# Stylish-TTS/stylish-tts

Hardware: AMD Instinct MI355X
Metric: audio frames/sec/GPU (24 kHz) forward+backward; DDP scaling 1/2/4/8 MI355X (higher is better)
Workload: dtype bf16 GEMM operands, f32 accumulation/storage; 1 GPU; c3: B=32/GPU T=520 frames (6.5 s) L=100

## Files before the change

stylish_tts_amd/csrc/bwd.hip:

```cpp
#include "sty_common.h"

namespace sty {

__device__ __forceinline__ double wave_sum(double v) {
  for (int o = 32; o > 0; o >>= 1) v += __shfl_xor(v, o);
  return v;
}

template <int N>
__device__ __forceinline__ void block_sum(double (&v)[N], double (*red)[4]) {
  const int lane = threadIdx.x & 63, wave = threadIdx.x >> 6;
#pragma unroll
  for (int i = 0; i < N; ++i) {
    v[i] = wave_sum(v[i]);
    if (lane == 0) red[i][wave] = v[i];
  }
  __syncthreads();
  if (threadIdx.x == 0) {
#pragma unroll
    for (int i = 0; i < N; ++i) v[i] = red[i][0] + red[i][1] + red[i][2] + red[i][3];
  }
}

__global__ __launch_bounds__(256) void pro_bwd_kernel(int mode_, const float* __restrict__ u, int Cu, int cu0,
// ... 542 lines not shown
  const float om = (in && out_mask) ? out_mask[(size_t)b * T + t] : 1.f;
  float mean = 0.f;
#pragma unroll
  for (int c = 0; c < 32; ++c) mean += xv[c];
  mean *= (1.0f / 32.0f);
  float var = 0.f;
#pragma unroll
  for (int c = 0; c < 32; ++c) {
    xv[c] -= mean;
    var = fmaf(xv[c], xv[c], var);
  }
  const float r = 1.0f / sqrtf(var * (1.0f / 32.0f) + eps);
  float s1 = 0.f, s2 = 0.f;
#pragma unroll
  for (int c = 0; c < 32; ++c) {
    xv[c] *= r;
    gv[c] *= om;
    const float dxh = gv[c] * A_s[c];
    s1 += dxh;
    s2 = fmaf(dxh, xv[c], s2);
  }
  s1 *= (1.0f / 32.0f);
  s2 *= (1.0f / 32.0f);
  if (in) {
#pragma unroll
    for (int c = 0; c < 32; ++c) {
      const float d = r * (gv[c] * A_s[c] - s1 - xv[c] * s2);
      if (h16 & 4) {
        sty_st_any(dx, base + (size_t)c * T, d, true);
      } else {
        float* o = reinterpret_cast<float*>(dx) + base + (size_t)c * T;
        *o = accumulate ? *o + d : d;
      }
    }
  }
#pragma unroll
  for (int c = 0; c < 32; ++c) {
    const float a0 = sty_half_sum_to_lane31(gv[c] * xv[c]);
    const float a1 = sty_half_sum_to_lane31(gv[c]);
    if ((tid & 31) == 31) {
      atomicAdd(&red[c], a0);
      atomicAdd(&red[32 + c], a1);
    }
  }
  __syncthreads();
  if (tid < 64) part[((size_t)b * gridDim.x + blockIdx.x) * 64 + tid] = red[tid];
}
__global__ __launch_bounds__(64) void chan_ln32_param_sum_kernel(const float* __restrict__ part, int B, int nblk, int ada,
                                                                 float* __restrict__ dgb, float* __restrict__ dw,
                                                                 float* __restrict__ db) {
  const int i = blockIdx.x, lane = threadIdx.x;
  const int slot = ada ? (i & 63) : i, b0 = ada ? i >> 6 : 0, nb = ada ? 1 : B;
  double s = 0.0;
  for (int b = b0; b < b0 + nb; ++b)
    for (int k = lane; k < nblk; k += 64) s += (double)part[((size_t)b * nblk + k) * 64 + slot];
  s = wave_sum(s);
  if (lane == 0) {
    if (ada)
      dgb[(size_t)b0 * 64 + slot] += (float)s;
    else if (slot < 32)
      dw[slot] += (float)s;
    else
      db[slot - 32] += (float)s;
  }
}

__global__ void cast_any_kernel(const void* __restrict__ x, size_t n, void* __restrict__ y, int to16) {
  const size_t i = (size_t)blockIdx.x * 256 + threadIdx.x;
  if (i < n) sty_st_any(y, i, sty_ld_any(x, i, !to16), to16);
}
int launch_cast_f32_to_16(const float* x, size_t n, void* y16, hipStream_t st) {
  hipLaunchKernelGGL(cast_any_kernel, dim3((unsigned)((n + 255) / 256)), dim3(256), 0, st, x, n, y16, 1);
  STY_LAUNCH_CHECK();
  return STY_OK;
}
int launch_cast_16_to_f32(const void* x16, size_t n, float* y, hipStream_t st) {
  hipLaunchKernelGGL(cast_any_kernel, dim3((unsigned)((n + 255) / 256)), dim3(256), 0, st, x16, n, y, 0);
  STY_LAUNCH_CHECK();
  return STY_OK;
}
bool chan_ln32_eligible(int B, int C, int T, int relu) {
  return C == 32 && !relu && (size_t)B * T >= 65536 && getenv("STY_NO_LN32_BWD") == nullptr;
}
int launch_chan_ln_bwd(const float* x, const float* dy, const float* y, int B, int C, int T, float eps, int ada,
                       const float* w, const float* gb, int relu, const float* out_mask, float* dx, int accumulate,
                       float* mu_tmp, float* r_tmp, float* dgb, float* dw, float* db, hipStream_t st, int h16) {
  const bool no32 = getenv("STY_NO_LN32_BWD") != nullptr;
  if (C == 32 && !relu && (size_t)B * T >= 65536 && !no32) {
    const int nblk = cdiv(T, 256);
    if ((h16 & 4) && accumulate) {
      set_error("chan_ln_bwd: a two-byte dx cannot be accumulated into");
      return STY_EINVAL;
    }
    hipLaunchKernelGGL(chan_ln32_bwd_kernel, dim3(nblk, B), dim3(256), 0, st, x, dy, T, eps, ada, w, gb, out_mask, dx, accumulate,
                       mu_tmp, h16);
    hipLaunchKernelGGL(chan_ln32_param_sum_kernel, dim3(ada ? B * 64 : 64), dim3(64), 0, st, mu_tmp, B, nblk, ada, dgb, dw, db);
    STY_LAUNCH_CHECK();
    return STY_OK;
  }
  if (h16) {
    set_error("chan_ln_bwd: two-byte tensors only on the C = 32 long-row kernel (chan_ln32_eligible)");
    return STY_EINVAL;
  }
  if ((size_t)B * T < 65536 && C <= 256)
    hipLaunchKernelGGL((chan_ln_bwd_dx_reg_kernel<16, 16>), dim3(cdiv(T, 16), B), dim3(256), 0, st, x, dy, y, C, T, eps, ada, w,
                       gb, relu, out_mask, dx, accumulate, mu_tmp, r_tmp);
  else if ((size_t)B * T >= 65536)
    hipLaunchKernelGGL(chan_ln_bwd_dx_kernel<64>, dim3(cdiv(T, 64), B), dim3(256), 0, st, x, dy, y, C, T, eps, ada, w, gb,
                       relu, out_mask, dx, accumulate, mu_tmp, r_tmp);
  else
    hipLaunchKernelGGL(chan_ln_bwd_dx_kernel<16>, dim3(cdiv(T, 16), B), dim3(256), 0, st, x, dy, y, C, T, eps, ada, w, gb,
                       relu, out_mask, dx, accumulate, mu_tmp, r_tmp);
  hipLaunchKernelGGL(chan_ln_bwd_param_kernel, dim3(C, B), dim3(256), 0, st, x, dy, y, mu_tmp, r_tmp, C, T, ada, relu,
                     out_mask, dgb, dw, db);
  STY_LAUNCH_CHECK();
  return STY_OK;
}

__global__ __launch_bounds__(256) void grn_bwd_kernel(const double* __restrict__ part, int nseg,
                                                      const float* __restrict__ gamma,
                                                      const float* __restrict__ ds, int C4,
                                                      float* __restrict__ coef, float* __restrict__ dgamma) {
  __shared__ float gxs[1024];
  __shared__ double red[2][4];
  const int b = blockIdx.x;
  if (nseg < 32) {
    for (int c = threadIdx.x; c < C4; c += 256) {
      double sq = 0.0;
      for (int k = 0; k < nseg; ++k) sq += part[(((size_t)b * C4 + c) * nseg + k) * 2 + 1];
      gxs[c] = (float)sqrt(sq);
    }
  } else {
    const int lane = threadIdx.x & 63, wave = threadIdx.x >> 6;
    for (int c = wave; c < C4; c += 4) {
      const double* pp = part + ((size_t)b * C4 + c) * nseg * 2 + 1;
      double sq = 0.0;
      for (int k = lane; k < nseg; k += 64) sq += pp[(size_t)k * 2];
      for (int o = 32; o > 0; o >>= 1) sq += __shfl_xor(sq, o);
      if (lane == 0) gxs[c] = (float)sqrt(sq);
    }
  }
  __syncthreads();
  double acc[1] = {0.0};
  for (int c = threadIdx.x; c < C4; c += 256) acc[0] += gxs[c];
  __shared__ float mean_s, dot_s;
  block_sum<1>(acc, red);
  if (threadIdx.x == 0) mean_s = (float)(acc[0] / C4);
  __syncthreads();
  const float m = mean_s + 1e-6f;
  double d2[1] = {0.0};
  for (int c = threadIdx.x; c < C4; c += 256) {
    const float dnx = ds[(size_t)b * C4 + c] * gamma[c];
    d2[0] += (double)dnx * gxs[c];
    atomicAdd(&dgamma[c], ds[(size_t)b * C4 + c] * (gxs[c] / m));
  }
  __syncthreads();
  block_sum<1>(d2, red);
  if (threadIdx.x == 0) dot_s = (float)d2[0];
  __syncthreads();
  for (int c = threadIdx.x; c < C4; c += 256) {
    const float dnx = ds[(size_t)b * C4 + c] * gamma[c];
    const float dgx = dnx / m - dot_s / (m * m) / (float)C4;
    coef[(size_t)b * C4 + c] = gxs[c] > 0.f ? dgx / gxs[c] : 0.f;
  }
}
int launch_grn_bwd(const double* part, int nseg, const float* gamma, const float* ds, int B, int C4, float* coef,
                   float* dgamma, hipStream_t st) {
  if (C4 > 1024) {
    set_error("grn_bwd: 4C > 1024");
    return STY_EINVAL;
  }
  hipLaunchKernelGGL(grn_bwd_kernel, dim3(B), dim3(256), 0, st, part, nseg, gamma, ds, C4, coef, dgamma);
  STY_LAUNCH_CHECK();
  return STY_OK;
}

__global__ void act_fwd_kernel(int kind, const float* __restrict__ x, const float* __restrict__ alpha, int C, int T,
                               float* __restrict__ y) {
  const int t = blockIdx.x * 256 + threadIdx.x, c = blockIdx.y, b = blockIdx.z;
  if (t >= T) return;
  if (kind == ACT_GLU) {
    const float a = x[((size_t)b * 2 * C + c) * T + t], g = x[((size_t)b * 2 * C + C + c) * T + t];
    y[((size_t)b * C + c) * T + t] = a / (1.f + expf(-g));
    return;
  }
  const size_t o = ((size_t)b * C + c) * T + t;
  const float v = x[o];
  float r = v;
  if (kind == ACT_RELU) r = fmaxf(v, 0.f);
  else if (kind == ACT_SWISH) r = v / (1.f + expf(-v));
  else if (kind == ACT_SNAKE) r = sty_snake(v, alpha[c], 1.f / alpha[c]);
  else if (kind == 100) r = tanhf(v);
  else if (kind == ACT_GELU) r = 0.5f * v * (1.0f + erff(v * 0.70710678118654752f));
  y[o] = r;
}
__device__ __forceinline__ float act_apply1(int kind, float v, float al, float ral) {
  float r = v;
// ... 787 lines not shown
```

stylish_tts_amd/csrc/model.h:

```cpp
#pragma once
#include <string>
#include <unordered_map>
#include <vector>

#include "sty_common.h"

namespace sty {

struct Param {
  const float* p = nullptr;
  std::vector<int64_t> shape;
};

int convnext32_ntiles(int T);
int launch_convnext32(const Cnx32Args& a, int B, int pass, hipStream_t st);
int launch_pack_w2a(const float* w2, const float* b2, const float* grn_beta, int C, float* w2a, float* b2eff,
                    hipStream_t st);
int launch_attention(const AttnArgs& a, int B, int DH, hipStream_t st);
int launch_rope_n(float* q, float* k, int B, int H, int DH, int L, int d, hipStream_t st, float sgn = 1.0f);
int launch_style_expand(const float* style, int B, int S, int L, float* y, hipStream_t st);
int launch_row_sum_add(const float* src, int rows, int L, float* dst, hipStream_t st);
int launch_wn_dw_bwd(const float* dw, const float* g, const float* v, int C, int K, float* dg, float* dv, hipStream_t st);
int launch_dur_post_bwd(const float* d, const float* mask, const float* go, int B, int NC, int L, float* gd, hipStream_t st);
int trainer_duration_forward(struct Trainer* t, int B, int L, const int64_t* texts, const int64_t* lengths, const float* style,
// ... 159 lines not shown
  int heads = 2;
};

struct Trainer;
struct StyleResBlk {
  int Cin = 0, Cout = 0;
  bool down = false, has_sc = false;
  PackedConv c1, c2, sc;
  const float* dw_w9 = nullptr;
  const float* dw_b = nullptr;
};
struct StylePlan {
  int n_mels = 80, style_dim = 64;
  PackedConv stem;
  StyleResBlk blk[4];
  PackedConv head;
  const float *fc_w = nullptr, *fc_b = nullptr;
};

}

struct sty_model {
  std::string kind;
  std::unordered_map<std::string, sty::Param> params;
  std::vector<std::string> requested;
  bool finalized = false, prepared = false;
  bool train_prepared = false;
  hipEvent_t prepared_ev = nullptr;
  int style_dim = 64;
  char* arena = nullptr;
  size_t arena_bytes = 0;
  sty::Bump ab;
  std::vector<sty::PackJob> jobs;
  std::vector<sty::StyleFcDesc> fcs;
  sty::StyleFcDesc* fcs_dev = nullptr;
  size_t gb_floats_per_batch = 0;
  std::string missing;
  sty::VocoderPlan voc;
  sty::TextEncPlan te;
  sty::DecoderPlan dec;
  sty::StylePlan sty_enc;
  sty::DurationPlan dur;
  sty::PitchEnergyPlan pe;
  sty::PackedConv pse_pre;
  float* stft_default = nullptr;
  bool train_enabled = false;
  char* garena = nullptr;
  std::unordered_map<const float*, float*> pgrad;
  std::unordered_map<std::string, float*> pgrad_by_key;
  std::unordered_map<const float*, sty::PackedConv> dgrad;
  std::unordered_map<const float*, sty::PackedConv> plain_of;
  void* fcs_bwd_dev = nullptr;
  sty::MultiJob* mj_dev[5] = {nullptr, nullptr, nullptr, nullptr, nullptr};
  int* mj_blk_dev[5] = {nullptr, nullptr, nullptr, nullptr, nullptr};
  int mj_nblk[5] = {0, 0, 0, 0, 0};
  int* mj_blk1_dev = nullptr;
  int mj_nblk1 = 0, mj_nsn = 0;
  bool mj_ready = false;
  size_t seg_job_split = 0;
  int seg_blk_split = 0;
  sty_grad_hook grad_hook = nullptr;
  void* grad_hook_user = nullptr;
  sty_train_opts topts = {0, 0, 0, 0, 0.1f, 0u, 0.2f, 0, 0};
  struct sty::Trainer* trainer = nullptr;
};

#include <functional>
#include <unordered_set>
namespace sty {
int launch_pro_bwd(int mode, const float* u, int Cu, int cu0, const float* x, int B, int C, int T, const float* pa,
                   const float* ps, int pC, int pc0, const float* alpha, const float* mask, float* dx, int accumulate,
                   float* dpa, float* dps, float* dalpha, hipStream_t st);
int launch_adain_fold_bwd(const float* da, const float* ds, const float* mean, const float* rstd, const float* gb, int B,
                          int C, int T, float* dgb, float* c0, float* c1, hipStream_t st);
int launch_row_axpb(const float* x, const float* c0, const float* c1, int rows, int T, float* dx, hipStream_t st);
int launch_pro_bwd_adain(const void* u, int uh, const void* x, int xh, int B, int C, int T, const float* pa, const float* ps,
                         const float* alpha, const float* mean, const float* rstd, const float* gb, void* dx, int dh,
                         int accumulate, float* dgb, float* dalpha, int hw, hipStream_t st, const void* dsrc = nullptr);
int launch_adain_stats(const double* part, int nseg, int rows, int T, float eps, float* mean, float* rstd,
                       hipStream_t st);
int launch_cast_f32_to_16(const float* x, size_t n, void* y16, hipStream_t st);
int launch_cast_16_to_f32(const void* x16, size_t n, float* y, hipStream_t st);
bool chan_ln32_eligible(int B, int C, int T, int relu);
int launch_chan_ln_bwd(const float* x, const float* dy, const float* y, int B, int C, int T, float eps, int ada,
                       const float* w, const float* gb, int relu, const float* out_mask, float* dx, int accumulate,
                       float* mu_tmp, float* r_tmp, float* dgb, float* dw, float* db, hipStream_t st, int h16 = 0);
int launch_grn_bwd(const double* part, int nseg, const float* gamma, const float* ds, int B, int C4, float* coef,
                   float* dgamma, hipStream_t st);
int launch_act_fwd(int kind, const float* x, const float* alpha, int B, int C, int T, float* y, hipStream_t st);
int launch_act_bwd(int kind, const float* x, const float* dy, const float* alpha, int B, int C, int T, float* dx,
                   int accumulate, float* dalpha, hipStream_t st);
int launch_row_scale_add(const float* src, const float* coef, float k, int rows, int T, float* dst, hipStream_t st);
int launch_dwconv_fwd(const float* x, const float* w, const float* bias, int B, int C, int T, int K, int pad, float* y,
                      hipStream_t st);
size_t dwconv_bwd_scratch_floats(int B, int C, int T, int K);
int launch_dwconv_bwd(const float* x, const float* dy, const float* w, int B, int C, int T, int K, int pad, float* dx,
                      int accumulate, float* dw, float* db, float* scratch, hipStream_t st, const float* dx_src = nullptr,
                      int x16 = 0, int dy16 = 0);
int launch_bn_eval_fwd(const float* x, const float* w, const float* b, const float* rm, const float* rv, float eps,
                       int B, int C, int T, float* y, hipStream_t st);
int launch_bn_eval_bwd(const float* x, const float* dy, const float* w, const float* rm, const float* rv, float eps,
                       int B, int C, int T, float* dx, float* dw, float* db, hipStream_t st);
size_t bias_grad_scratch_floats(int B, int C, int T);
int launch_bias_grad(const float* g, const float* mask, int B, int C, int T, int shuffle, float scale, float* db,
                     float* scratch, hipStream_t st);
int launch_style_fc_bwd(const void* descs_dev, int nlayers, int B, int style_dim, const float* style,
                        const float* dgb_base, float* dstyle, hipStream_t st);
int launch_istft64_bwd(int B, int F, const float* audio, const float* daudio, const float* logamp, const float* real,
                       const float* imag, const float* bbr, const float* bbi, float* dlogamp, float* dreal,
                       float* dimag, hipStream_t st);
size_t wgrad_partial_floats(const PackedConv& w, int B, int T);
struct WgReduceDefer;
WgReduceDefer* wgrad_defer_create();
void wgrad_defer_destroy(WgReduceDefer* d);
WgReduceDefer* wgrad_defer_set(WgReduceDefer* d);
size_t wgrad_defer_pending(const WgReduceDefer* d);
int wgrad_defer_flush(WgReduceDefer* d, int site, hipStream_t st);
inline bool wgrad_fuses_bias(const PackedConv& w) { return w.K <= 12; }
int launch_conv1d_wgrad(const ConvArgs& fwd, const float* g, const float* gmask, float scale, float* gwp,
                        float* partial, float* gbias, bool* bias_done, hipStream_t st);
bool conv1d_wgrad_reads_twins_only(const ConvArgs& fwd, bool gmask);
int launch_pack_dgrad(const float* wp, int K, int CinP, int CoutP, float* wd, hipStream_t st);
int launch_b2eff_bwd(const float* g, const float* w2, const float* beta, int C, float* db2, float* dbeta, float* dW2,
                     hipStream_t st);
int launch_unpack_grad(const float* gwp, const float* g, const float* v, int Cout, int Cin, int K, int CinP, int CoutP,
                       int glu, float* dW, float* dg, float* dv, hipStream_t st);
int launch_attention_bwd(const AttnArgs& a, const float* dO, float* dQ, float* dK, float* dV, size_t dqbs, size_t dkbs,
                         size_t dvbs, size_t dobs, int B, int DH, float* ws, hipStream_t st, int overwrite = 0);
bool attention_bwd_can_overwrite(const AttnArgs& a, int DH);
bool attention_bwd_mfma_dh(int DH);
size_t attention_bwd_ws_floats(int B, int H, int T);
int launch_rope_signed(float* q, float* k, int B, int H, int DH, int L, int d, const float* theta4, float sgn,
                       hipStream_t st);
int launch_embedding_bwd(const int64_t* tokens, const float* g, int B, int L, int H, int ntok, float scale, float* demb,
                         hipStream_t st);
int launch_bmm_ct_bwd(const float* g, const float* ali, int B, int C, int L, int T, float* denc, hipStream_t st);
int launch_slice_add(const float* src, int Csrc, int c0, int B, int C, int T, float* dst, hipStream_t st);
int launch_fnv_bwd(const float* pitch, const float* energy, const float* voiced, const float* w34, const float* g, int B,
                   int T, float* dw34, float* dp, float* de, float* dv, hipStream_t st);
int launch_fnv_unpack(const float* dw34, const float* g0, const float* v0, const float* g1, const float* v1,
                      const float* g2, const float* v2, float* dg0, float* dv0, float* db0, float* dg1, float* dv1,
                      float* db1, float* dg2, float* dv2, float* db2, hipStream_t st);
int launch_pack_dgrad2d(const float* wp, int KW, int KH, int Cin, int Cout, int CinP, int CoutP, int CinPd, int CoutPd,
                        float* wd, hipStream_t st);
size_t dwconv2d_s2_bwd_scratch_floats(int B, int C, int H, int W);
int launch_dwconv2d_s2_bwd(const float* x, const float* gy, const float* gate, const float* w9, int B, int C, int H, int W, float* dx,
                           int accumulate, float* dw9, float* db, float* scratch, hipStream_t st, __bf16* dx16 = nullptr,
                           const float* mask16 = nullptr);
int launch_pad_cols(const float* x, size_t rows, int W, float* y, hipStream_t st);
int launch_flat_mask(int B, int H, int Wp, int Hv, int Wv, float* m, hipStream_t st);
int launch_dw2d_sn_unpack(const float* g9, const float* w, const float* u, const float* v, const float* t, int C,
                          float* dW, hipStream_t st);
int launch_avgpool2_bwd(const float* gy, int BC, int H, int W, float scale, float* dx, const float* gate, hipStream_t st,
                        __bf16* dx16 = nullptr, const float* mask16 = nullptr, int C = 0);
int launch_pool_fc_bwd(const float* x, int B, int C, int n, int count, const float* W, int S, const float* gs,
                       float* dW, float* db, float* dx, int accumulate, hipStream_t st);
int launch_bn_train_fwd(const float* x, const float* w, const float* b, float* rm, float* rv, float eps, float momentum,
                        int B, int C, int T, float* y, float* mean, float* rstd, double* part, hipStream_t st);
int launch_bn_train_bwd(const float* x, const float* dy, const float* w, const float* mean, const float* rstd, int B,
                        int C, int T, float* dx, int accumulate, float* dw, float* db, float* sums, hipStream_t st);
int launch_dropout(const float* x, const float* res, size_t n, float p, unsigned seed, unsigned site, float* y,
                   int accumulate, hipStream_t st, size_t group = 1);
int launch_box_smooth(const float* x, int B, int T, int width, float* y, int accumulate, hipStream_t st);
size_t sn_power_iter_scratch_floats(int Cout, int n);
int trainer_style_forward(struct Trainer* t, int B, int T, const float* mel, float* style, void* ws, size_t ws_bytes,
                          hipStream_t st, size_t* need, const float* pitch = nullptr, const float* energy = nullptr);
int trainer_style_backward(struct Trainer* t, const float* d_style, hipStream_t st);
int trainer_style_tap(struct Trainer* t, int i, int grad, float* dst, int* C, int* H, int* W, hipStream_t st);
struct Trainer;
// ... 21 lines not shown
```

stylish_tts_amd/csrc/sty_common.h:

```cpp
#pragma once
#include <hip/hip_runtime.h>
#include <stdint.h>
#include <stdio.h>

#include "../../include/stylish_hip.h"

namespace sty {

void set_error(const char* fmt, ...);
int hip_fail(hipError_t e, const char* what);

#define STY_HIP(expr)                                      \
  do {                                                     \
    hipError_t _e = (expr);                                \
    if (_e != hipSuccess) return sty::hip_fail(_e, #expr); \
  } while (0)

#define STY_LAUNCH_CHECK() STY_HIP(hipGetLastError())

extern thread_local const void* g_last_kernel;
template <class R, class... A>
inline const void* kernel_handle(R (*f)(A...)) {
  return reinterpret_cast<const void*>(f);
}
// ... 30 lines not shown
  r[6] = (__bf16)v6;
  r[7] = (__bf16)v7;
  return r;
}
#endif

#ifdef __HIPCC__
typedef __bf16 bf16x2 __attribute__((ext_vector_type(2)));
__device__ __forceinline__ float sty_bf_lo(unsigned u) { return __builtin_bit_cast(float, u << 16); }
__device__ __forceinline__ float sty_bf_hi(unsigned u) { return __builtin_bit_cast(float, u & 0xffff0000u); }
__device__ __forceinline__ unsigned sty_pack2_bf16(float lo, float hi) {
  bf16x2 r;
  r[0] = (__bf16)lo;
  r[1] = (__bf16)hi;
  return __builtin_bit_cast(unsigned, r);
}
__device__ __forceinline__ float sty_round_bf16(float v) {
  return __builtin_bit_cast(float, (unsigned)__builtin_bit_cast(unsigned short, (__bf16)v) << 16);
}
__device__ __forceinline__ float sty_ld_any(const void* p, size_t i, bool h) {
  return h ? sty_bf_lo(reinterpret_cast<const unsigned short*>(p)[i]) : reinterpret_cast<const float*>(p)[i];
}
__device__ __forceinline__ void sty_st_any(void* p, size_t i, float v, bool h) {
  if (h)
    reinterpret_cast<unsigned short*>(p)[i] = __builtin_bit_cast(unsigned short, (__bf16)v);
  else
    reinterpret_cast<float*>(p)[i] = v;
}
__device__ __forceinline__ float4 sty_ld4_any(const void* p, size_t i4, bool h) {
  if (h) {
    const uint2 u = reinterpret_cast<const uint2*>(p)[i4];
    return make_float4(sty_bf_lo(u.x), sty_bf_hi(u.x), sty_bf_lo(u.y), sty_bf_hi(u.y));
  }
  return reinterpret_cast<const float4*>(p)[i4];
}
__device__ __forceinline__ void sty_st4_any(void* p, size_t i4, float4 v, bool h) {
  if (h)
    reinterpret_cast<uint2*>(p)[i4] = make_uint2(sty_pack2_bf16(v.x, v.y), sty_pack2_bf16(v.z, v.w));
  else
    reinterpret_cast<float4*>(p)[i4] = v;
}
#endif

static inline int cdiv(int a, int b) { return (a + b - 1) / b; }
#ifdef __HIPCC__
__device__ __forceinline__ int wg_chunks(int mode, int split, int nsplit, int total, int& first, int& end) {
  if (mode == 1) {
    first = (int)(((long long)split * total) / nsplit);
    end = (int)(((long long)(split + 1) * total) / nsplit);
    return 1;
  }
  end = total;
  if (mode == 2) {
    const int k = split & 7, q = nsplit >> 3, r = nsplit & 7;
    first = k * q + (k < r ? k : r) + (split >> 3);
  } else {
    first = split;
  }
  return nsplit;
}
#endif

static inline size_t align_up(size_t v, size_t a) { return (v + a - 1) / a * a; }

struct PackedConv {
  const float* wp = nullptr;
  const float* bias = nullptr;
  int Cin = 0, Cout = 0, K = 1, CinP = 0, CoutP = 0;
  const void* wf = nullptr;
};

constexpr int CI_CHUNK = 32;

enum ConvPro : int {
  PRO_NONE = 0,
  PRO_AFFINE = 1,
  PRO_AFFINE_SNAKE = 2,
  PRO_AFFINE_LRELU = 3,
  PRO_LN_AFFINE = 4,
  PRO_MASK = 5,
  PRO_SCALE = 6,
  PRO_LRELU = 7,
};
enum ConvAct : int { ACT_NONE = 0, ACT_RELU = 1, ACT_SWISH = 2, ACT_SNAKE = 3, ACT_GLU = 4, ACT_GELU = 5,
                     ACT_LRELU01 = 6 };

struct ConvArgs {
  const float* x[3] = {nullptr, nullptr, nullptr};
  int xc[3] = {0, 0, 0};
  int nsrc = 1;
  int B = 0, T = 0;
  int Tin = 0;
  int dil = 1, pad = 0;
  int hpad = 0, Cin2d = 0;
  int flatW = 0;
  int ksplit_max = 4;
  int bf16 = 0;
  int in_shuffle = 0;
  PackedConv w;
  int pro = PRO_NONE;
  const float* pa = nullptr;
  const float* ps = nullptr;
  const float* palpha = nullptr;
  const float* pbeta = nullptr;
  float ln_eps = 1e-6f;
  const float* mask = nullptr;
  int act = ACT_NONE;
  const float* act_alpha = nullptr;
  float out_scale = 1.f;
  const float* residual = nullptr;
  const float* out_mask = nullptr;
  int out_mask_post = 0;
  int shuffle = 1;
  int ln_out = 0;
  const float* ln_w = nullptr;
  const float* ln_b = nullptr;
  float* y = nullptr;
  float* y_split = nullptr;
  double* stat_part = nullptr;
  const __bf16* x16 = nullptr;
  const __bf16* g16 = nullptr;
  __bf16* y16 = nullptr;
  int y16_act = PRO_NONE;
  const float* up_g = nullptr;
  const __bf16* up_gate16 = nullptr;
  const float* up_mask = nullptr;
  float up_scale = 1.f;
  int up_H = 0;
  int xh = 0, yh = 0, rh = 0, gh = 0;
  int w_row = 0, w_tap = 0;
};
int launch_twin_cast(const float* x, const float* mask, int pro, int B, int C, int T, __bf16* y16, hipStream_t st);
bool wgradb16_eligible(const ConvArgs& fwd);
int launch_wgradb16(const ConvArgs& fwd, int nsplit, float* partial, int want_bias, hipStream_t st);

int launch_conv1d(const ConvArgs& a, hipStream_t st);
bool conv1d_reads_twin_only(const ConvArgs& a);
bool conv1d_has_up_stage(const ConvArgs& a);
bool conv32p_eligible(const ConvArgs& a);
int conv32p_stat_nseg(int T);
bool wgradb_eligible(const ConvArgs& fwd, bool gmask);
int launch_wgradb(const ConvArgs& ax, const ConvArgs& ag, int nsplit, float* partial, int want_bias, hipStream_t st);
int wgradb_chunks(const PackedConv& w, int B, int T, int dil);
bool wgradp32_eligible(const ConvArgs& fwd);
int wgradp32_chunks(const ConvArgs& fwd);
int launch_wgradp32(const ConvArgs& ax, const ConvArgs& ag, int nsplit, float* partial, int want_bias, hipStream_t st);
int wgrad_cnx_nsplit(int B, int T);
int launch_conv_wgrad_cnx(int x_wide, const void* wide, const float* narrow, int B, int T, float* gwp, float* partial,
                          float* gbias, hipStream_t st, int narrow16 = 0);
int wgrad_cnx_per_b(int B, int T);
int launch_wgrad_cnx(int x_wide, const void* wide, const float* narrow, int B, int T, float* partial, int want_bias,
                     hipStream_t st, int per_b = 0, int narrow16 = 0);
bool stem2d_eligible(const ConvArgs& a);
int launch_stem2d(const ConvArgs& a, hipStream_t st);
bool convk1_eligible(const ConvArgs& a);
int launch_convk1(const ConvArgs& a, hipStream_t st);
bool convp16_eligible(const ConvArgs& a);
bool convq_eligible(const ConvArgs& a);
int launch_convq(const ConvArgs& a, hipStream_t st);
int convp16_repack_range(const void* lo, const void* hi, hipStream_t st);
void convp16_forget_range(const void* lo, const void* hi);
int launch_convp16(const ConvArgs& a, hipStream_t st);
int launch_conv32p(const ConvArgs& a, hipStream_t st);

struct MultiJob {
  const float *p0 = nullptr, *p1 = nullptr, *p2 = nullptr, *p3 = nullptr, *p4 = nullptr;
// ... 303 lines not shown
```

stylish_tts_amd/csrc/train.hip:

```cpp
#include <stdlib.h>
#include <string.h>

#include <map>
#include <memory>
#include <unordered_map>

#include "model.h"

namespace sty {

struct Trainer {
  sty_model* m = nullptr;
  hipStream_t st = nullptr;
  int B = 0, T = 0;
  Bump ws;
  int rc = STY_OK;
  float* gb = nullptr;
  float* dgb = nullptr;
  const float* style = nullptr;
  float* audio = nullptr;
  std::vector<std::function<void()>> tape;
  std::unordered_map<const float*, float*> gmap;
  std::unordered_set<const float*> nograd;
  float* scratch_param = nullptr;
  size_t scratch_param_n = 0;
  const float* mel_in = nullptr;
  size_t peak = 0;

  bool dry = false;
  bool live() const { return !dry && ws.base != nullptr && rc == STY_OK; }
  void chk(int r) {
    if (rc == STY_OK && r != STY_OK) rc = r;
  }

  std::vector<char> fcs_bwd_sent;
  hipStream_t st2 = nullptr;
  bool side_on = getenv("STY_NO_SIDE_STREAM") == nullptr;
  std::vector<hipEvent_t> evs;
  size_t ev_used = 0;
  std::unordered_set<const float*> side_reads;
  bool side_dirty = false;
  size_t side_need = 0;
  float* side_partial = nullptr;
  WgReduceDefer* defer = wgrad_defer_create();
  bool defer_on = getenv("STY_NO_DEFERRED_REDUCE") == nullptr;
  size_t wg_sum = 0, wg_off = 0;
  float* wg_base = nullptr;
  int flush_site = 0;
  std::vector<std::function<void(hipStream_t)>> after_reduce;
  bool deferring() const { return wg_base != nullptr; }
  float* wg_take(size_t n) {
    n = (n + 63) & ~size_t(63);
    float* p = wg_base + wg_off;
    wg_off += n;
    if (wg_off > wg_sum && rc == STY_OK) {
      set_error("training: weight-gradient partial region too small (%zu > %zu floats)", wg_off, wg_sum);
      rc = STY_ESTATE;
    }
    return p;
  }
  void wg_need(size_t n) { wg_sum += (n + 63) & ~size_t(63); }
  struct DeferScope {
    WgReduceDefer* old;
    explicit DeferScope(Trainer* t) { old = wgrad_defer_set(t->deferring() && t->live() ? t->defer : nullptr); }
    ~DeferScope() { (void)wgrad_defer_set(old); }
  };
  void reduce_flush(hipStream_t s) {
    if (!deferring() || !live()) {
      after_reduce.clear();
      return;
    }
    chk(wgrad_defer_flush(defer, flush_site++, s));
    WgReduceDefer* cur = wgrad_defer_set(nullptr);
    if (rc == STY_OK)
      for (auto& fn : after_reduce) fn(s);
    (void)wgrad_defer_set(cur);
    after_reduce.clear();
  }
  bool twins_env = getenv("STY_NO_TWINS") == nullptr;
  bool twins_on() const { return twins_env && m->topts.compute_bf16 != 0; }
  std::unordered_map<const float*, __bf16*> tw_x[2];
  std::unordered_set<const float*> tw_want;
  std::unordered_map<const float*, std::pair<__bf16*, const float*>> tw_g;
  static int tw_slot(int pro) { return pro == PRO_LRELU ? 1 : 0; }
  void twin_register(const float* x, int pro, __bf16* t) { tw_x[tw_slot(pro)][x] = t; }
  const __bf16* xtwin(const float* x, int pro, int C, int n) {
    auto& mp = tw_x[tw_slot(pro)];
    auto it = mp.find(x);
    if (it != mp.end()) return it->second;
    __bf16* t = take<__bf16>((size_t)B * C * n);
    if (live()) chk(launch_twin_cast(x, nullptr, pro, B, C, n, t, st));
    mp[x] = t;
    return t;
  }
  std::unordered_set<const float*> g_twin_only, g_no_fp32;
  struct LazyMask {
    const float* src;
    const float* mask;
    int C, n;
    float* dst;
  };
  std::unordered_map<const float*, LazyMask> lazy_mask;
  bool mask_pending(const float* act) const { return !lazy_mask.empty() && lazy_mask.count(act) != 0; }
  void mask_flush(const float* act) {
    auto it = lazy_mask.find(act);
    if (it == lazy_mask.end()) return;
    const LazyMask z = it->second;
    lazy_mask.erase(it);
    if (live())
      chk(launch_pro_bwd(PRO_MASK, z.src, z.C, 0, z.src, B, z.C, z.n, nullptr, nullptr, z.C, 0, nullptr, z.mask, z.dst, 0,
                         nullptr, nullptr, nullptr, st));
  }
  struct PendUp {
    const float* g;
    const float* mask;
    float scale;
    int BC, C, H, W, n;
  };
  std::unordered_map<const float*, PendUp> pend_up;
  void up_apply(const float* src, const PendUp& u) {
// ... 202 lines not shown
    a.y = y;
    a.bf16 = m->topts.compute_bf16;
    return a;
  }

  void conv(const ConvArgs& a0) {
    ConvArgs a = a0;
    a.bf16 = m->topts.compute_bf16;
    a.xh = is16(a.x[0]);
    a.yh = is16(a.y);
    a.rh = is16(a.residual);
    if (a.nsrc > 1 && (is16(a.x[1]) || is16(a.x[2]))) {
      set_error("training: a bf16-stored tensor as source 1 / 2 of a channel-concatenated conv");
      rc = STY_ESTATE;
      return;
    }
    const size_t pn = wgrad_partial_floats(a.w, B, a.T);
    side_need = pn > side_need ? pn : side_need;
    wg_need(pn);
    if (live()) chk(launch_conv1d(a, st));
    ConvArgs f = a;
    tape.push_back([this, f]() { conv_bwd(f); });
  }
  void conv_bwd(const ConvArgs& f) {
    const PackedConv& w = f.w;
    const int Tt = f.T;
    const size_t ny = (size_t)B * w.Cout * Tt;
    float* gY = G(f.y, ny);
    float* gR = nullptr;
    if (f.residual && wants(f.residual)) {
      if (!gmap.count(f.residual) && !(f.out_mask && f.out_mask_post) && f.shuffle <= 1)
        gmap[f.residual] = gY;
      else
        gR = G(f.residual, ny);
    }
    float* gX[3] = {nullptr, nullptr, nullptr};
    int accX[3] = {1, 1, 1};
    bool any = false;
    const float* gX_src = nullptr;
    if (f.nsrc == 1 && f.pro == PRO_AFFINE_SNAKE && Tt % 8 == 0 && wants(f.x[0]) && !side_reads.empty()) {
      auto ia = adain_of.find(f.pa);
      auto ig = gmap.find(f.x[0]);
      if (ia != adain_of.end() && ia->second.x == f.x[0] && ia->second.s == f.ps && !*ia->second.done && ig != gmap.end() &&
          side_reads.count(ig->second) && !is16(ig->second) && (ungated.empty() || !ungated.count(f.x[0]))) {
        gX_src = ig->second;
        gX[0] = take<float>((size_t)B * f.xc[0] * Tt);
        gmap[f.x[0]] = gX[0];
        accX[0] = 1;
        any = true;
      }
    }
    for (int i = 0; i < f.nsrc; ++i)
      if (wants(f.x[i]) && !(i == 0 && gX_src)) {
        gX[i] = Gw(f.x[i], (size_t)B * f.xc[i] * Tt, accX[i]);
        any = true;
      }
    for (int i = 1; i < f.nsrc; ++i)
      for (int j = 0; j < i; ++j)
        if (gX[i] && gX[i] == gX[j]) accX[i] = 1;
    if (side_ready())
      for (int i = 0; i < f.nsrc; ++i)
        if (gX[i] && gX[i] == gY) gX[i] = fresh_copy(f.x[i], gY, (size_t)B * f.xc[i] * Tt);
    float* dpa = nullptr;
    float* dps = nullptr;
    float* dal = nullptr;
    AdainInfo* fuse = nullptr;
    if (any && f.pro == PRO_AFFINE_SNAKE && f.nsrc == 1 && Tt % 8 == 0) {
      auto it = adain_of.find(f.pa);
      if (it != adain_of.end() && it->second.x == f.x[0] && it->second.s == f.ps && !*it->second.done) fuse = &it->second;
    }
    if (any && fuse) {
      dal = PG(f.palpha, w.Cin);
    } else if (any) {
      if (f.pro == PRO_AFFINE_SNAKE || f.pro == PRO_AFFINE_LRELU || f.pro == PRO_AFFINE) {
        int dummy;
        dpa = Gw(f.pa, (size_t)B * w.Cin, dummy);
        dps = Gw(f.ps, (size_t)B * w.Cin, dummy);
      } else if (f.pro == PRO_SCALE) {
        int dummy;
        dpa = Gw(f.pa, (size_t)B * w.Cin, dummy);
      }
      if (f.pro == PRO_AFFINE_SNAKE) dal = PG(f.palpha, w.Cin);
    }
    const size_t mark = ws.off;
    const float* gmask = f.out_mask;
    if (gR && live()) {
      if (f.out_mask && f.out_mask_post)
        chk(launch_pro_bwd(PRO_MASK, gY, w.Cout, 0, gY, B, w.Cout, Tt, nullptr, nullptr, w.Cout, 0, nullptr, f.out_mask,
                           gR, 1, nullptr, nullptr, nullptr, st));
      else
        chk(launch_row_scale_add(gY, nullptr, 1.0f, B * w.Cout, Tt, gR, st));
    }
    bool bias_done = false;
    float* gbias = w.bias ? PGpacked(w.bias) : nullptr;
    if (m->topts.frozen) {
      bias_done = true;
    } else if (side_ready()) {
      float* sp = deferring() ? wg_take(wgrad_partial_floats(w, B, Tt)) : side_partial;
      float* gwp = PGpacked(w.wp);
      const float osc = f.out_scale;
      side_push(gY, [=](hipStream_t s) { chk(launch_conv1d_wgrad(f, gY, gmask, osc, gwp, sp, gbias, nullptr, s)); });
      bias_done = wgrad_fuses_bias(w);
    } else {
      const size_t pn = wgrad_partial_floats(w, B, Tt);
      float* partial = deferring() ? wg_take(pn) : take<float>(pn);
      DeferScope ds(this);
      if (live()) chk(launch_conv1d_wgrad(f, gY, gmask, f.out_scale, PGpacked(w.wp), partial, gbias, &bias_done, st));
    }
    if (w.bias && !bias_done) {
      float* bs = take<float>(bias_grad_scratch_floats(B, w.Cout, Tt));
      if (live()) chk(launch_bias_grad(gY, gmask, B, w.Cout, Tt, f.shuffle, f.out_scale, PGpacked(w.bias), bs, st));
    }
    if (any) {
      auto it = m->dgrad.find(w.wp);
      if (it == m->dgrad.end()) {
        set_error("training: no input-gradient weights for a conv (model not finalized for training?)");
        rc = STY_ESTATE;
        return;
      }
      const bool u16 = f.xh && f.nsrc == 1 && act16_on();
      float* U = take_act((size_t)B * w.Cin * Tt, u16);
      struct UGuard {
        Trainer* t;
        float* U;
        size_t mark;
        ~UGuard() {
          t->half_.erase(U);
          t->ws.off = mark;
        }
      } u_guard{this, U, mark};
      ConvArgs d;
      d.x[0] = gY;
      d.xc[0] = w.Cout;
      d.nsrc = 1;
      d.B = B;
      d.T = Tt;
      d.w = it->second;
      d.dil = f.dil;
      d.bf16 = f.bf16;
      d.pad = (w.K - 1) * f.dil - f.pad;
      d.out_scale = f.out_scale;
      d.in_shuffle = f.shuffle > 1 ? f.shuffle : 0;
      if (gmask) {
        d.pro = PRO_MASK;
        d.mask = gmask;
      }
      d.y = U;
      d.yh = u16;
      d.xh = is16(gY);
      if (f.nsrc == 1 && (f.pro == PRO_NONE || f.pro == PRO_MASK) && gX[0] != gY) {
        d.y = gX[0];
        d.yh = is16(gX[0]);
        d.rh = d.yh;
        d.residual = accX[0] ? gX[0] : nullptr;
        if (f.pro == PRO_MASK) {
          d.out_mask = f.mask;
          d.out_mask_post = 0;
        }
        if (live()) chk(launch_conv1d(d, st));
        ws.off = mark;
        return;
      }
      if (live()) chk(launch_conv1d(d, st));
      if (fuse) {
        *fuse->done = true;
        if (live())
          chk(launch_pro_bwd_adain(U, u16, f.x[0], f.xh, B, w.Cin, Tt, f.pa, f.ps, f.palpha, fuse->mean, fuse->rstd, fuse->gbl,
                                   gX[0], is16(gX[0]), accX[0], fuse->dgl, dal, f.bf16 ? 1 : 0, st, gX_src));
        half_.erase(U);
        ws.off = mark;
        return;
      }
      if (gX_src) {
        set_error("training: out-of-place prologue backward planned without the fused kernel");
        rc = STY_ESTATE;
        return;
      }
      if (u16 || f.xh) {
        half_.erase(U);
        set_error("training: bf16-stored conv input without the fused prologue backward");
        rc = STY_ESTATE;
        return;
      }
      int c0 = 0;
      for (int i = 0; i < f.nsrc; ++i) {
        if (gX[i] && live())
          chk(launch_pro_bwd(f.pro | (f.bf16 ? 0x100 : 0), U, w.Cin, c0, f.x[i], B, f.xc[i], Tt, f.pa, f.ps, w.Cin, c0, f.palpha, f.mask, gX[i],
                             accX[i], dpa, dps, dal, st));
        c0 += f.xc[i];
      }
    }
    ws.off = mark;
  }

  float* act(int kind, const float* x, const float* alpha, int C, int Tt) {
    float* y = take<float>((size_t)B * C * Tt);
    if (live()) chk(launch_act_fwd(kind, x, alpha, B, C, Tt, y, st));
    tape.push_back([=]() {
      const int Cin = kind == ACT_GLU ? 2 * C : C;
      float* gY = G(y, (size_t)B * C * Tt);
      int acc = 1;
      float* gX = Gw(x, (size_t)B * Cin * Tt, acc);
      float* dal = kind == ACT_SNAKE ? PG(alpha, C) : nullptr;
      if (live()) chk(launch_act_bwd(kind, x, gY, alpha, B, C, Tt, gX, acc, dal, st));
    });
    return y;
  }

  unsigned drop_site = 0;
  bool dropout_on() const { return m->topts.dropout_seed != 0; }
  float* dropout(const float* x, float p, int C, int Tt, const float* residual, size_t group = 1) {
    const size_t n = (size_t)B * C * Tt;
    float* y = take<float>(n);
    const unsigned seed = m->topts.dropout_seed, site = drop_site++;
    if (live()) chk(launch_dropout(x, residual, n, p, seed, site, y, 0, st, group));
    tape.push_back([=]() {
      float* gY = G(y, n);
      if (residual && wants(residual)) {
        if (!gmap.count(residual)) {
          gmap[residual] = gY;
        } else {
          float* gR = G(residual, n);
          if (live()) chk(launch_row_scale_add(gY, nullptr, 1.0f, 1, (int)n, gR, st));
        }
      }
      int acc = 1;
      float* gX = Gw(x, n, acc);
      if (gX == gY) {
        set_error("dropout backward: aliased gradient buffers");
        rc = STY_ESTATE;
        return;
      }
      if (live()) chk(launch_dropout(gY, nullptr, n, p, seed, site, gX, acc, st, group));
    });
    return y;
  }

  float* layernorm(const float* x, int C, int Tt, float eps, const AdaFc* fc, const float* w, const float* bvec,
                   int relu = 0, const float* omask = nullptr) {
    float* y = take<float>((size_t)B * C * Tt);
    const float* gbl = fc ? gbp(*fc) : nullptr;
    float* dgl = fc ? dgbp(*fc) : nullptr;
    if (live()) chk(launch_chan_layernorm(x, y, B, C, Tt, eps, fc ? 1 : 0, w, bvec, gbl, relu, omask, st));
    const bool ln32 = grad16_on() && chan_ln32_eligible(B, C, Tt, relu);
    if (ln32 && grad16_stream_on()) g16_ok.insert(y);
    tape.push_back([=]() {
      const size_t nel = (size_t)B * C * Tt;
      float* gY = ln32 ? G16(y, nel) : G(y, nel);
      int acc = 1, h16 = is16(gY) ? 2 : 0;
      float* gX;
      if (ln32 && g16_ok.count(x) && !gmap.count(x)) {
        gX = take_act(nel, true);
        gmap[x] = gX;
        acc = 0;
        h16 |= 4;
      } else {
        gX = Gw(x, nel, acc);
      }
      const size_t mark = ws.off;
      float* mu = take<float>((size_t)B * Tt);
      float* r = take<float>((size_t)B * Tt);
      float* dw = fc ? nullptr : PG(w, C);
      float* db = fc ? nullptr : PG(bvec, C);
      if (live())
        chk(launch_chan_ln_bwd(x, gY, y, B, C, Tt, eps, fc ? 1 : 0, w, gbl, relu, omask, gX, acc, mu, r, dgl, dw, db, st, h16));
      ws.off = mark;
    });
    return y;
  }

  struct AdainInfo {
    const float *x, *s, *mean, *rstd, *gbl;
    float* dgl;
    std::shared_ptr<bool> done;
  };
  std::unordered_map<const float*, AdainInfo> adain_of;
  void adain(const float* x, int C, int Tt, const AdaFc& fc, float*& a, float*& s, const double* have_part = nullptr,
             int have_nseg = 0) {
    a = take<float>((size_t)B * C);
    s = take<float>((size_t)B * C);
    float* mean = take<float>((size_t)B * C);
    float* rstd = take<float>((size_t)B * C);
    const int nseg = have_part ? have_nseg : row_stats_nseg(Tt);
    const double* part = have_part;
    if (!have_part) {
      double* p2 = take<double>((size_t)B * C * nseg * 2);
      if (live()) chk(launch_row_stats(x, B * C, Tt, p2, st));
      part = p2;
    }
    if (live()) {
      chk(launch_adain_finalize(part, nseg, gbp(fc), B, C, Tt, 1e-5f, a, s, st));
      chk(launch_adain_stats(part, nseg, B * C, Tt, 1e-5f, mean, rstd, st));
    }
    const float* gbl = gbp(fc);
    float* dgl = dgbp(fc);
    float* aa = a;
    float* ss = s;
    auto done = std::make_shared<bool>(false);
    adain_of[aa] = AdainInfo{x, ss, mean, rstd, gbl, dgl, done};
    if (!have_part && is16(x)) {
      set_error("training: instance-norm statistics pass over a bf16-stored tensor (the producing conv leaves them behind)");
      rc = STY_ESTATE;
    }
    tape.push_back([=]() {
      if (*done) return;
      if (is16(x)) {
        set_error("training: AdaIN backward over a bf16-stored tensor outside the fused prologue backward");
        rc = STY_ESTATE;
        return;
      }
      float* da = G(aa, (size_t)B * C);
      float* ds = G(ss, (size_t)B * C);
      float* gX = G(x, (size_t)B * C * Tt);
      const size_t mark = ws.off;
      float* c0 = take<float>((size_t)B * C);
      float* c1 = take<float>((size_t)B * C);
      if (live()) {
        chk(launch_adain_fold_bwd(da, ds, mean, rstd, gbl, B, C, Tt, dgl, c0, c1, st));
        chk(launch_row_axpb(x, c0, c1, B * C, Tt, gX, st));
      }
      ws.off = mark;
    });
  }

  float* dwconv(const float* x, const float* w, const float* bias, int C, int Tt, int K, int pad) {
    float* y = take<float>((size_t)B * C * Tt);
    if (live()) chk(launch_dwconv_fwd(x, w, bias, B, C, Tt, K, pad, y, st));
    tape.push_back([=]() {
      float* gY = G(y, (size_t)B * C * Tt);
      int acc = 1;
      float* gX = wants(x) ? Gw(x, (size_t)B * C * Tt, acc) : nullptr;
      float* gw = PG(w, (size_t)C * K);
      float* gb = PG(bias, C);
      if (side_ready() && gX != gY) {
        float* sc = take<float>(dwconv_bwd_scratch_floats(B, C, Tt, K));
        side_push(gY, [=](hipStream_t s2) {
          chk(launch_dwconv_bwd(x, gY, w, B, C, Tt, K, pad, nullptr, 0, gw, gb, sc, s2));
        });
        if (live() && gX) chk(launch_dwconv_bwd(x, gY, w, B, C, Tt, K, pad, gX, acc, nullptr, nullptr, nullptr, st));
        return;
      }
      const size_t mark = ws.off;
      float* sc = take<float>(dwconv_bwd_scratch_floats(B, C, Tt, K));
      if (live()) chk(launch_dwconv_bwd(x, gY, w, B, C, Tt, K, pad, gX, acc, gw, gb, sc, st));
      ws.off = mark;
    });
// ... 2064 lines not shown
```

Baseline: 381,600 frames/s.

## Move leaf parameter-gradient kernels (conv bias, LayerNorm params) onto side stream

Conv bias-gradient reductions are pushed to the side stream alongside the weight-gradient kernel. Non-ada channel LayerNorm backward is split so dx runs on the main stream and the parameter sums run on the side stream. Both target overlapping leaf gradient work with the critical input-gradient path. This adds cross-stream dependencies and keeps mu/r scratch alive past the main-stream call (the early return skips resetting the workspace mark), which risks memory growth or lifetime bugs.

```diff
diff --git a/stylish_tts_amd/csrc/bwd.hip b/stylish_tts_amd/csrc/bwd.hip
--- a/stylish_tts_amd/csrc/bwd.hip
+++ b/stylish_tts_amd/csrc/bwd.hip
@@ -648,12 +648,17 @@
 bool chan_ln32_eligible(int B, int C, int T, int relu) {
   return C == 32 && !relu && (size_t)B * T >= 65536 && getenv("STY_NO_LN32_BWD") == nullptr;
 }
+bool chan_ln_bwd_is_split(int B, int C, int T, int relu) { return !chan_ln32_eligible(B, C, T, relu); }
 int launch_chan_ln_bwd(const float* x, const float* dy, const float* y, int B, int C, int T, float eps, int ada,
                        const float* w, const float* gb, int relu, const float* out_mask, float* dx, int accumulate,
-                       float* mu_tmp, float* r_tmp, float* dgb, float* dw, float* db, hipStream_t st, int h16) {
+                       float* mu_tmp, float* r_tmp, float* dgb, float* dw, float* db, hipStream_t st, int h16, int parts) {
   const bool no32 = getenv("STY_NO_LN32_BWD") != nullptr;
   if (C == 32 && !relu && (size_t)B * T >= 65536 && !no32) {
     const int nblk = cdiv(T, 256);
+    if (parts != LN_BWD_BOTH) {
+      set_error("chan_ln_bwd: the long-row kernel computes dx and the parameter sums in one pass");
+      return STY_EINVAL;
+    }
     if ((h16 & 4) && accumulate) {
       set_error("chan_ln_bwd: a two-byte dx cannot be accumulated into");
       return STY_EINVAL;
@@ -668,7 +673,8 @@
     set_error("chan_ln_bwd: two-byte tensors only on the C = 32 long-row kernel (chan_ln32_eligible)");
     return STY_EINVAL;
   }
-  if ((size_t)B * T < 65536 && C <= 256)
+  if (!(parts & LN_BWD_DX)) {
+  } else if ((size_t)B * T < 65536 && C <= 256)
     hipLaunchKernelGGL((chan_ln_bwd_dx_reg_kernel<16, 16>), dim3(cdiv(T, 16), B), dim3(256), 0, st, x, dy, y, C, T, eps, ada, w,
                        gb, relu, out_mask, dx, accumulate, mu_tmp, r_tmp);
   else if ((size_t)B * T >= 65536)
@@ -677,8 +683,9 @@
   else
     hipLaunchKernelGGL(chan_ln_bwd_dx_kernel<16>, dim3(cdiv(T, 16), B), dim3(256), 0, st, x, dy, y, C, T, eps, ada, w, gb,
                        relu, out_mask, dx, accumulate, mu_tmp, r_tmp);
-  hipLaunchKernelGGL(chan_ln_bwd_param_kernel, dim3(C, B), dim3(256), 0, st, x, dy, y, mu_tmp, r_tmp, C, T, ada, relu,
-                     out_mask, dgb, dw, db);
+  if (parts & LN_BWD_PARAM)
+    hipLaunchKernelGGL(chan_ln_bwd_param_kernel, dim3(C, B), dim3(256), 0, st, x, dy, y, mu_tmp, r_tmp, C, T, ada, relu,
+                       out_mask, dgb, dw, db);
   STY_LAUNCH_CHECK();
   return STY_OK;
 }
diff --git a/stylish_tts_amd/csrc/model.h b/stylish_tts_amd/csrc/model.h
--- a/stylish_tts_amd/csrc/model.h
+++ b/stylish_tts_amd/csrc/model.h
@@ -265,9 +265,11 @@
 int launch_cast_f32_to_16(const float* x, size_t n, void* y16, hipStream_t st);
 int launch_cast_16_to_f32(const void* x16, size_t n, float* y, hipStream_t st);
 bool chan_ln32_eligible(int B, int C, int T, int relu);
+bool chan_ln_bwd_is_split(int B, int C, int T, int relu);
 int launch_chan_ln_bwd(const float* x, const float* dy, const float* y, int B, int C, int T, float eps, int ada,
                        const float* w, const float* gb, int relu, const float* out_mask, float* dx, int accumulate,
-                       float* mu_tmp, float* r_tmp, float* dgb, float* dw, float* db, hipStream_t st, int h16 = 0);
+                       float* mu_tmp, float* r_tmp, float* dgb, float* dw, float* db, hipStream_t st, int h16 = 0,
+                       int parts = LN_BWD_BOTH);
 int launch_grn_bwd(const double* part, int nseg, const float* gamma, const float* ds, int B, int C4, float* coef,
                    float* dgamma, hipStream_t st);
 int launch_act_fwd(int kind, const float* x, const float* alpha, int B, int C, int T, float* y, hipStream_t st);
diff --git a/stylish_tts_amd/csrc/sty_common.h b/stylish_tts_amd/csrc/sty_common.h
--- a/stylish_tts_amd/csrc/sty_common.h
+++ b/stylish_tts_amd/csrc/sty_common.h
@@ -136,6 +136,7 @@
   PRO_SCALE = 6,
   PRO_LRELU = 7,
 };
+enum { LN_BWD_DX = 1, LN_BWD_PARAM = 2, LN_BWD_BOTH = 3 };
 enum ConvAct : int { ACT_NONE = 0, ACT_RELU = 1, ACT_SWISH = 2, ACT_SNAKE = 3, ACT_GLU = 4, ACT_GELU = 5,
                      ACT_LRELU01 = 6 };
 
diff --git a/stylish_tts_amd/csrc/train.hip b/stylish_tts_amd/csrc/train.hip
--- a/stylish_tts_amd/csrc/train.hip
+++ b/stylish_tts_amd/csrc/train.hip
@@ -36,6 +36,8 @@
   std::vector<char> fcs_bwd_sent;
   hipStream_t st2 = nullptr;
   bool side_on = getenv("STY_NO_SIDE_STREAM") == nullptr;
+  bool leaf_side_env = getenv("STY_NO_LEAF_SIDE") == nullptr;
+  bool leaf_side() const { return leaf_side_env && side_ready(); }
   std::vector<hipEvent_t> evs;
   size_t ev_used = 0;
   std::unordered_set<const float*> side_reads;
@@ -404,6 +406,9 @@
       }
       if (f.pro == PRO_AFFINE_SNAKE) dal = PG(f.palpha, w.Cin);
     }
+    float* bs_side = nullptr;
+    if (w.bias && !m->topts.frozen && leaf_side() && !wgrad_fuses_bias(w))
+      bs_side = take<float>(bias_grad_scratch_floats(B, w.Cout, Tt));
     const size_t mark = ws.off;
     const float* gmask = f.out_mask;
     if (gR && live()) {
@@ -421,8 +426,12 @@
       float* sp = deferring() ? wg_take(wgrad_partial_floats(w, B, Tt)) : side_partial;
       float* gwp = PGpacked(w.wp);
       const float osc = f.out_scale;
-      side_push(gY, [=](hipStream_t s) { chk(launch_conv1d_wgrad(f, gY, gmask, osc, gwp, sp, gbias, nullptr, s)); });
-      bias_done = wgrad_fuses_bias(w);
+      const int shuf = f.shuffle, Co = w.Cout;
+      side_push(gY, [=](hipStream_t s) {
+        chk(launch_conv1d_wgrad(f, gY, gmask, osc, gwp, sp, gbias, nullptr, s));
+        if (bs_side) chk(launch_bias_grad(gY, gmask, B, Co, Tt, shuf, osc, gbias, bs_side, s));
+      });
+      bias_done = wgrad_fuses_bias(w) || bs_side != nullptr;
     } else {
       const size_t pn = wgrad_partial_floats(w, B, Tt);
       float* partial = deferring() ? wg_take(pn) : take<float>(pn);
@@ -584,6 +593,14 @@
       float* r = take<float>((size_t)B * Tt);
       float* dw = fc ? nullptr : PG(w, C);
       float* db = fc ? nullptr : PG(bvec, C);
+      if (!fc && leaf_side() && !h16 && gX != gY && chan_ln_bwd_is_split(B, C, Tt, relu)) {
+        if (live())
+          chk(launch_chan_ln_bwd(x, gY, y, B, C, Tt, eps, 0, w, gbl, relu, omask, gX, acc, mu, r, dgl, dw, db, st, 0, LN_BWD_DX));
+        side_push(gY, [=](hipStream_t s2) {
+          chk(launch_chan_ln_bwd(x, gY, y, B, C, Tt, eps, 0, w, gbl, relu, omask, gX, acc, mu, r, dgl, dw, db, s2, 0, LN_BWD_PARAM));
+        });
+        return;
+      }
       if (live())
         chk(launch_chan_ln_bwd(x, gY, y, B, C, Tt, eps, fc ? 1 : 0, w, gbl, relu, omask, gX, acc, mu, r, dgl, dw, db, st, h16));
       ws.off = mark;
```

Result: no change. 384,200 frames/s, median of 6 (+0.7%).
